# redradman/MujocoPoseLearning

Measured on AMD Instinct MI355X. Metric: env steps/sec (whole node), humanoid 'stand' task, 1/2/4/8 MI355X, higher is better.
Workload: dtype f64

## Files before the change

### mujocoposelearning_amd/csrc/hs_lanes.h

```cpp
#pragma once
#include <hip/hip_runtime.h>

#include <cstdint>
#include <type_traits>

#include "hs_kernels.h"
#include "hs_model.h"

namespace hs {
namespace {

constexpr int WAVE = 64;
constexpr int HL = 32;
static_assert(MAXDOF == HL, "one dof per sub-lane (lim_row slots, dof masks)");

template <int NCON, int NEFC, bool W = false, bool LT = false>
struct Cap {
  static constexpr int CON = NCON;
  static constexpr int EFC = NEFC;
  static constexpr int RPL = NEFC / HL;
  static constexpr bool WIDE = W;
  static constexpr bool LANES = LT;
  static constexpr bool NEAR = LT;
  static_assert((NCON % HL == 0 || HL % NCON == 0) && NEFC % HL == 0, "capacity in whole half-waves");
};
template <typename T>
using Resident = std::conditional_t<sizeof(T) == 8, Cap<MAXCON_F64, MAXEFC_F64, false, true>, Cap<MAXCON, MAXEFC>>;
using Wide = Cap<MAXCON_WIDE, MAXEFC_WIDE, true>;

#define SCHED_FENCE() __builtin_amdgcn_sched_barrier(0)

#define WSYNC() asm volatile("" ::: "memory")

template <int B, int E, typename F>
__device__ __forceinline__ void static_for(F&& f) {
  if constexpr (B < E) {
    f(std::integral_constant<int, B>{});
    static_for<B + 1, E>(f);
  }
}
template <int CTRL>
__device__ __forceinline__ uint32_t dpp32(uint32_t v) {
  return (uint32_t)__builtin_amdgcn_mov_dpp((int)v, CTRL, 0xF, 0xF, true);
}
struct RowPair { uint32_t lo, hi; };
__device__ __forceinline__ RowPair rowswap(uint32_t v) {
  auto r = __builtin_amdgcn_permlane16_swap(v, v, false, false);
  return {r[0], r[1]};
}
template <int K>
__device__ __forceinline__ uint32_t bcast32(uint32_t v) {
  RowPair r = rowswap(dpp32<0x150 + (K & 15)>(v));
  return K < 16 ? r.lo : r.hi;
}
template <int K>
__device__ __forceinline__ float bcast(float v) {
  return __uint_as_float(bcast32<K>(__float_as_uint(v)));
}
template <int K>
__device__ __forceinline__ double bcast(double v) {
  uint64_t x = (uint64_t)__double_as_longlong(v);
  uint64_t lo = bcast32<K>((uint32_t)x), hi = bcast32<K>((uint32_t)(x >> 32));
  return __longlong_as_double((long long)((hi << 32) | lo));
}
template <int CTRL>
__device__ __forceinline__ float dpp(float v) {
  return __uint_as_float(dpp32<CTRL>(__float_as_uint(v)));
}
template <int CTRL>
__device__ __forceinline__ double dpp(double v) {
  uint64_t x = (uint64_t)__double_as_longlong(v);
  uint64_t lo = dpp32<CTRL>((uint32_t)x), hi = dpp32<CTRL>((uint32_t)(x >> 32));
  return __longlong_as_double((long long)((hi << 32) | lo));
}
__device__ __forceinline__ float rows_sum(float v) {
  RowPair r = rowswap(__float_as_uint(v));
  return __uint_as_float(r.lo) + __uint_as_float(r.hi);
}
__device__ __forceinline__ double rows_sum(double v) {
  uint64_t x = (uint64_t)__double_as_longlong(v);
  RowPair l = rowswap((uint32_t)x), h = rowswap((uint32_t)(x >> 32));
  return __longlong_as_double((long long)(((uint64_t)h.lo << 32) | l.lo)) +
         __longlong_as_double((long long)(((uint64_t)h.hi << 32) | l.hi));
}
__device__ __forceinline__ float up_row(float v) { return __uint_as_float(rowswap(__float_as_uint(v)).hi); }
__device__ __forceinline__ double up_row(double v) {
  uint64_t x = (uint64_t)__double_as_longlong(v);
  const uint64_t lo = rowswap((uint32_t)x).hi, hi = rowswap((uint32_t)(x >> 32)).hi;
  return __longlong_as_double((long long)((hi << 32) | lo));
}
template <typename T>
__device__ __forceinline__ T hsum(T v) {
  v += dpp<0xB1>(v);
  v += dpp<0x4E>(v);
  v += dpp<0x141>(v);
  v += dpp<0x140>(v);
  return rows_sum(v);
}
__device__ __forceinline__ uint32_t hballot(bool p, bool upper) {
  uint64_t m = __ballot(p);
  return upper ? (uint32_t)(m >> 32) : (uint32_t)m;
}
template <typename T, bool AHEAD = false, typename LD, typename F>
__device__ __forceinline__ void for_bits(uint32_t mk, LD&& ld, F&& f) {
  if constexpr (AHEAD) {
    if (mk == 0u) return;
    int j = __builtin_ctz(mk);
    mk &= mk - 1u;
    auto cur = ld(j);
    for (; mk; mk &= mk - 1u) {
      const int jn = __builtin_ctz(mk);
      auto nxt = ld(jn);
      f(j, cur);
      cur = nxt;
      j = jn;
    }
    f(j, cur);
  } else {
    for (; mk; mk &= mk - 1u) {
      const int j = __builtin_ctz(mk);
      f(j, ld(j));
    }
  }
}
template <typename T, int N>
struct Vals { T v[N]; };
template <typename T, int N>
struct ValsX { T x; T v[N]; };

template <typename P>
__device__ __forceinline__ P opaque(P p) {
  uint64_t v = (uint64_t)p;
  uint32_t lo = __builtin_amdgcn_readfirstlane((uint32_t)v), hi = __builtin_amdgcn_readfirstlane((uint32_t)(v >> 32));
  v = ((uint64_t)hi << 32) | lo;
  asm volatile("" : "+s"(v));
  return (P)v;
}
template <typename T>
using MPtr = const __attribute__((address_space(4))) DevModel<T>*;
template <typename T>
using CPtr = const __attribute__((address_space(4))) T*;
template <typename T>
__device__ __forceinline__ LaneTable<T>& lane_table() {
  __shared__ LaneTable<T> tab;
  return tab;
}
template <typename T>
__device__ __forceinline__ void load_lane_table(MPtr<T> m) {
  constexpr int N = (int)(sizeof(LaneTable<T>) / 16), PER = (N + WAVE - 1) / WAVE;
  static_assert(sizeof(LaneTable<T>) % 16 == 0 && alignof(LaneTable<T>) == 16, "16-byte pieces");
  typedef uint32_t Piece __attribute__((ext_vector_type(4)));
  CPtr<Piece> src = (CPtr<Piece>)&m->lanes;
  Piece* dst = reinterpret_cast<Piece*>(&lane_table<T>());
  const int lane = threadIdx.x;
  Piece v[PER];
#pragma unroll
  for (int i = 0; i < PER; i++) {
    const int k = lane + i * WAVE;
    v[i] = src[k < N ? k : N - 1];
  }
#pragma unroll
  for (int i = 0; i < PER; i++) {
    const int k = lane + i * WAVE;
    if (k < N) dst[k] = v[i];
  }
  asm volatile("" ::: "memory");
}
template <typename C, typename T>
__device__ __forceinline__ decltype(auto) lanes(MPtr<T> m) {
  if constexpr (C::LANES) return (lane_table<T>());
  else return (*m);
}
#ifdef HS_ONLY_F32
#define HS_LT(C, m) (*(m))
#define HS_KTAIL(s) (s).u.k
#else
#define HS_LT(C, m) lanes<C>(m)
#define HS_KTAIL(s) (s).ktail()
#endif
template <typename T>
struct KArgs {
  MPtr<T> m;
  EnvBuffers<T> b;
  const float* actions;
  const uint8_t* reset_mask;
  const T* nz_q;
  const T* nz_v;
  StepParams p;
  int nenv;
  TapeOut<T> tape;
  RolloutArgs ro;
  EvalArgs ev;
  NormArgs nm;
  TermArgs tm;
};
template <typename T>
using KPtr = const __attribute__((address_space(4))) KArgs<T>*;
__device__ __forceinline__ int opaque_v(int x) {
  asm volatile("" : "+v"(x));
  return x;
}
__device__ __forceinline__ int below(uint32_t m, int sl) { return __popc(m & ((1u << sl) - 1u)); }
__device__ __forceinline__ bool bit(uint32_t mask, int i) { return i < 32 && ((mask >> i) & 1u); }
template <typename T>
__device__ __forceinline__ bool isbad(T x) {
  return !(x <= T(1e10) && x >= T(-1e10));
}

template <typename T>
__device__ __forceinline__ T row_ld(const T* p) {
  return __hip_atomic_load(const_cast<T*>(p), __ATOMIC_RELAXED, __HIP_MEMORY_SCOPE_AGENT);
}
template <typename T>
__device__ __forceinline__ void row_st(T* p, T v) {
  __hip_atomic_store(p, v, __ATOMIC_RELAXED, __HIP_MEMORY_SCOPE_AGENT);
}

__device__ __forceinline__ void sincos_t(double x, double& s, double& c) { sincos(x, &s, &c); }
__device__ __forceinline__ void sincos_t(float x, float& s, float& c) { s = __sinf(x); c = __cosf(x); }
template <typename T>
__device__ __forceinline__ void quat2mat(const T* q, T* R) {
  T w = q[0], x = q[1], y = q[2], z = q[3];
  R[0] = 1 - 2 * (y * y + z * z); R[1] = 2 * (x * y - w * z); R[2] = 2 * (x * z + w * y);
  R[3] = 2 * (x * y + w * z); R[4] = 1 - 2 * (x * x + z * z); R[5] = 2 * (y * z - w * x);
  R[6] = 2 * (x * z - w * y); R[7] = 2 * (y * z + w * x); R[8] = 1 - 2 * (x * x + y * y);
}
template <typename T>
__device__ __forceinline__ void mulq(const T* a, const T* b, T* r) {
  T t0 = a[0] * b[0] - a[1] * b[1] - a[2] * b[2] - a[3] * b[3];
  T t1 = a[0] * b[1] + a[1] * b[0] + a[2] * b[3] - a[3] * b[2];
  T t2 = a[0] * b[2] - a[1] * b[3] + a[2] * b[0] + a[3] * b[1];
  T t3 = a[0] * b[3] + a[1] * b[2] - a[2] * b[1] + a[3] * b[0];
  r[0] = t0; r[1] = t1; r[2] = t2; r[3] = t3;
}
template <typename T>
__device__ __forceinline__ void mv3(const T* R, const T* v, T* r) {
  T a = R[0] * v[0] + R[1] * v[1] + R[2] * v[2];
  T b = R[3] * v[0] + R[4] * v[1] + R[5] * v[2];
  T c = R[6] * v[0] + R[7] * v[1] + R[8] * v[2];
  r[0] = a; r[1] = b; r[2] = c;
}
template <typename T>
__device__ __forceinline__ void cross3(const T* a, const T* b, T* r) {
  T x = a[1] * b[2] - a[2] * b[1], y = a[2] * b[0] - a[0] * b[2], z = a[0] * b[1] - a[1] * b[0];
  r[0] = x; r[1] = y; r[2] = z;
}
template <typename T>
__device__ __forceinline__ T dot3(const T* a, const T* b) { return a[0] * b[0] + a[1] * b[1] + a[2] * b[2]; }
template <typename T>
__device__ __forceinline__ T dot6(const T* a, const T* b) {
  return a[0] * b[0] + a[1] * b[1] + a[2] * b[2] + a[3] * b[3] + a[4] * b[4] + a[5] * b[5];
}
template <typename T>
__device__ __forceinline__ T rsqrt_t(T x);
template <>
__device__ __forceinline__ float rsqrt_t<float>(float x) { return __builtin_amdgcn_rsqf(x); }
__device__ __forceinline__ float recip(float x) { return 1.0f / x; }
__device__ __forceinline__ double recip(double x) {
  double y = __builtin_amdgcn_rcp(x);
  const double e = fma(-x, y, 1.0);
  return fma(fma(e, e, e), y, y);
}
template <>
__device__ __forceinline__ double rsqrt_t<double>(double x) {
  const double y = __builtin_amdgcn_rsq(x);
  double g = x * y, h = 0.5 * y;
  const double r = fma(-h, g, 0.5);
  h = fma(h, r, h);
  const double y1 = h + h;
  const double e = fma(-(x * y1), y1, 1.0);
  return fma(h, e, y1);
}
template <typename T>
__device__ __forceinline__ T normalize3(T* v) {
  const T n2 = dot3(v, v);
  if (n2 < T(1e-30)) { v[0] = 1; v[1] = 0; v[2] = 0; return sqrt(n2); }
  const T i = rsqrt_t(n2);
  v[0] *= i; v[1] *= i; v[2] *= i;
  return n2 * i;
}
template <typename T>
__device__ __forceinline__ void normalize4(T* q) {
  const T n2 = q[0] * q[0] + q[1] * q[1] + q[2] * q[2] + q[3] * q[3];
  if (n2 < T(1e-30)) { q[0] = 1; q[1] = q[2] = q[3] = 0; }
  else { const T i = rsqrt_t(n2); q[0] *= i; q[1] *= i; q[2] *= i; q[3] *= i; }
}
template <typename T>
__device__ __forceinline__ void mul_inert(const T* i, const T* v, T* r) {
  r[0] = i[0] * v[0] + i[3] * v[1] + i[4] * v[2] - i[8] * v[4] + i[7] * v[5];
  r[1] = i[3] * v[0] + i[1] * v[1] + i[5] * v[2] + i[8] * v[3] - i[6] * v[5];
  r[2] = i[4] * v[0] + i[5] * v[1] + i[2] * v[2] - i[7] * v[3] + i[6] * v[4];
  r[3] = i[8] * v[1] - i[7] * v[2] + i[9] * v[3];
  r[4] = i[6] * v[2] - i[8] * v[0] + i[9] * v[4];
  r[5] = i[7] * v[0] - i[6] * v[1] + i[9] * v[5];
}
template <typename T>
__device__ __forceinline__ void cross_motion(const T* v, const T* m, T* r) {
  r[0] = -v[2] * m[1] + v[1] * m[2];
  r[1] = v[2] * m[0] - v[0] * m[2];
  r[2] = -v[1] * m[0] + v[0] * m[1];
  r[3] = -v[2] * m[4] + v[1] * m[5] - v[5] * m[1] + v[4] * m[2];
  r[4] = v[2] * m[3] - v[0] * m[5] + v[5] * m[0] - v[3] * m[2];
  r[5] = -v[1] * m[3] + v[0] * m[4] - v[4] * m[0] + v[3] * m[1];
}
template <typename T>
__device__ __forceinline__ void cross_force(const T* v, const T* f, T* r) {
  r[0] = -v[2] * f[1] + v[1] * f[2] - v[5] * f[4] + v[4] * f[5];
  r[1] = v[2] * f[0] - v[0] * f[2] + v[5] * f[3] - v[3] * f[5];
  r[2] = -v[1] * f[0] + v[0] * f[1] - v[4] * f[3] + v[3] * f[4];
  r[3] = -v[2] * f[4] + v[1] * f[5];
  r[4] = v[2] * f[3] - v[0] * f[5];
  r[5] = -v[1] * f[3] + v[0] * f[4];
}

}
}
```

### mujocoposelearning_amd/csrc/hs_scratch.h

```cpp
#pragma once
#include <cstdint>

#include "hs_lanes.h"
#include "hs_model.h"

namespace hs {
namespace {

enum RowKind { RK_JLO = 0, RK_JHI = 1, RK_TLO = 2, RK_THI = 3, RK_CN = 4, RK_P0 = 5 };
__device__ __forceinline__ int rk_kind(int kid) { return kid >> 16; }
__device__ __forceinline__ int rk_id(int kid) { return kid & 0xffff; }

template <typename T>
struct KinTail { T xanchor[MAXJNT][3]; T xaxis[MAXJNT][3]; T gpos[MAXGEOM][3]; T gax[MAXGEOM][3]; };

template <typename T, typename C>
struct Scratch {
  T qpos[MAXQ];
  T qvel[MAXDOF];
  T ctrl[MAXU];
  alignas(16) T vx[MAXDOF];
  T com[4];
  T cinert[MAXBODY][10];
  T cdof[MAXDOF][6];
  T cvel[MAXBODY][6];
  T con_pos[C::CON][3];
  T con_n[C::CON][3];
  T con_t1[C::CON][3];
  T con_dist[C::CON];
  T con_v[C::CON][3];
  T con_U[C::CON][6];
  T con_F[C::CON][3];
  int con_pair[C::CON];
  int con_adr[C::CON];
  uint32_t con_bb[C::CON];
  uint32_t con_m1[C::CON];
  uint32_t con_m2[C::CON];
  T con_mu[C::CON];
  uint32_t con_act[(C::CON + HL - 1) / HL];
  uint16_t lim_row[MAXDOF];
  uint32_t dense_mask[C::RPL];
  int row_kid[C::EFC];
  T row_D[C::EFC];
  T row_f[C::EFC];
  int ncon, nefc, nlim, njl;
  int niter;
  struct KinHead { T xpos[MAXBODY][3]; T xmat[MAXBODY][9]; T xquat[MAXBODY][4]; };
  struct KinFull { T xpos[MAXBODY][3]; T xmat[MAXBODY][9]; T xquat[MAXBODY][4]; T xanchor[MAXJNT][3];
                   T xaxis[MAXJNT][3]; T gpos[MAXGEOM][3]; T gax[MAXGEOM][3]; };
  using Kin = std::conditional_t<C::LANES, KinHead, KinFull>;
  static_assert(!C::LANES || sizeof(KinTail<T>) <= sizeof(T) * C::CON * 12, "KinTail fits con_v, con_U, con_F");
  __device__ __forceinline__ decltype(auto) ktail() {
    if constexpr (C::LANES) return (*reinterpret_cast<KinTail<T>*>(&con_v[0][0]));
    else return (u.k);
  }
  __device__ __forceinline__ decltype(auto) ktail() const {
    if constexpr (C::LANES) return (*reinterpret_cast<const KinTail<T>*>(&con_v[0][0]));
    else return (u.k);
  }
  static_assert(!C::NEAR || (C::LANES && sizeof(uint32_t) * MAXPAIR <= sizeof(T) * C::CON * 3 &&
                             sizeof(KinTail<T>) <= sizeof(T) * C::CON * 9),
                "the near-pair list fits con_F, past the KinTail over con_v / con_U");
  __device__ __forceinline__ uint32_t* near_list() { return reinterpret_cast<uint32_t*>(&con_F[0][0]); }
  union {
    Kin k;
    struct { T crb[MAXBODY][10]; T buf[MAXDOF][6]; } c;
    struct { T cdofdot[MAXDOF][6]; T cfrc[MAXBODY][6]; T csub[MAXBODY][6]; } r;
    struct { T bvel[MAXBODY][6];
             alignas(16) T cb[MAXDOF][2];
             T cfrc[MAXBODY][6], linv[MAXBODY][3], mv[MAXBODY][3]; } n;
    struct { alignas(16) float x[sizeof(T) == 8 ? 512 : 4]; alignas(16) float h[sizeof(T) == 8 ? 256 : 4]; } pol;
  } u;
};

constexpr int PGS_LA = 3;
template <typename T>
constexpr int pgs_cache_rows() { return sizeof(T) == 4 ? 40 : 48; }
template <typename T>
struct alignas(4 * sizeof(T)) PgsRow {
  T b, R, ar, ai;
  T g[4];
};
template <typename T, typename C>
struct PgsCache {
  static constexpr int NC = pgs_cache_rows<T>();
  T u[NC][MAXDOF];
  PgsRow<T> row[C::EFC];
};

}
}
```

### mujocoposelearning_amd/csrc/hs_stepper.h

```cpp
#pragma once
#include "hs_contacts.h"
#include "hs_dense.h"
#include "hs_lanes.h"
#include "hs_phase_clock.h"
#include "hs_scratch.h"

namespace hs {
namespace {

template <typename T, int NV, typename C>
struct Stepper {
  PhaseClock clk;
  MPtr<T> m;
  Scratch<T, C>& s;
  int sl, nb;
  bool up;
  T cd[6];
  T Mr[NV];
  T fsmooth;
  T fcon;
  T qacc;
  T qfa;
  T damp;
  int niter;
  T* dbg = nullptr;

  __device__ Stepper(MPtr<T> mm, Scratch<T, C>& ss, int lane)
      : m(mm), s(ss), sl(lane & (HL - 1)), nb(mm->nbody), up(lane >= HL) {}

  static constexpr bool LDLF = sizeof(T) == 8;
  static constexpr bool LDLE = false;
  __device__ __forceinline__ static KPtr<T> kargs() { return (KPtr<T>)__builtin_amdgcn_kernarg_segment_ptr(); }

  __device__ __forceinline__ void phase_begin() {
    m = opaque(m);
    sl = opaque_v(sl);
  }

  __device__ __forceinline__ void kinematics() {
    phase_begin();
    if (sl == 0) {
      for (int k = 0; k < 3; k++) s.u.k.xpos[0][k] = 0;
      s.u.k.xquat[0][0] = 1; s.u.k.xquat[0][1] = s.u.k.xquat[0][2] = s.u.k.xquat[0][3] = 0;
      for (int k = 0; k < 9; k++) s.u.k.xmat[0][k] = (k % 4 == 0) ? T(1) : T(0);
    }
    const int b = sl;
    const bool isb = b > 0 && b < nb;
    int depth = -1, par = 0, ja = 0, jn = 0, fqa = 0;
    bool isfree = false;
    T pl[3] = {0, 0, 0}, ql[4] = {1, 0, 0, 0};
    T anl[MAXJPB][3], axl[MAXJPB][3];
    if (isb) {
      depth = HS_LT(C, m).body_depth[b];
      par = HS_LT(C, m).body_parentid[b];
      ja = HS_LT(C, m).body_jntadr[b];
      jn = HS_LT(C, m).body_jntnum[b];
      isfree = jn == 1 && HS_LT(C, m).jnt_type[ja] == JNT_FREE;
      fqa = HS_LT(C, m).jnt_qposadr[ja];
      for (int k = 0; k < 3; k++) pl[k] = HS_LT(C, m).body_pos[b][k];
      for (int k = 0; k < 4; k++) ql[k] = HS_LT(C, m).body_quat[b][k];
    }
    if (isfree) {
      for (int k = 0; k < 3; k++) pl[k] = s.qpos[fqa + k];
      for (int k = 0; k < 4; k++) ql[k] = s.qpos[fqa + 3 + k];
    }
#pragma unroll
    for (int jj = 0; jj < MAXJPB; jj++) {
      const bool use = isb && !isfree && jj < jn;
      const int j = use ? ja + jj : 0;
      T jp[3], jx[3], ang = 0;
      for (int k = 0; k < 3; k++) { jp[k] = use ? m->jnt_pos[j][k] : T(0); jx[k] = use ? m->jnt_axis[j][k] : T(0); }
      if (use) {
        int qa = HS_LT(C, m).jnt_qposadr[j];
        ang = s.qpos[qa] - HS_LT(C, m).qpos0[qa];
      }
      T sn, cs;
      sincos_t(T(0.5) * ang, sn, cs);
      const T jr[4] = {cs, jx[0] * sn, jx[1] * sn, jx[2] * sn};
      T R[9];
      quat2mat(ql, R);
      mv3(R, jx, axl[jj]);
      mv3(R, jp, anl[jj]);
      for (int k = 0; k < 3; k++) anl[jj][k] += pl[k];
      if (use) {
        mulq(ql, jr, ql);
        quat2mat(ql, R);
        T v[3];
        mv3(R, jp, v);
        for (int k = 0; k < 3; k++) pl[k] = anl[jj][k] - v[k];
      }
    }
    WSYNC();
    for (int L = 1; L <= m->nlevel; L++) {
      if (depth == L) {
        T pos[3], q[4];
        if (isfree) {
          for (int k = 0; k < 3; k++) pos[k] = pl[k];
          for (int k = 0; k < 4; k++) q[k] = ql[k];
        } else {
          mv3(s.u.k.xmat[par], pl, pos);
          for (int k = 0; k < 3; k++) pos[k] += s.u.k.xpos[par][k];
          T pq[4] = {s.u.k.xquat[par][0], s.u.k.xquat[par][1], s.u.k.xquat[par][2], s.u.k.xquat[par][3]};
          mulq(pq, ql, q);
        }
        normalize4(q);
        for (int k = 0; k < 4; k++) s.u.k.xquat[b][k] = q[k];
        for (int k = 0; k < 3; k++) s.u.k.xpos[b][k] = pos[k];
        quat2mat(q, s.u.k.xmat[b]);
      }
      WSYNC();
    }
    if (isb) {
      if (isfree) {
        for (int k = 0; k < 3; k++) { HS_KTAIL(s).xanchor[ja][k] = s.u.k.xpos[b][k]; HS_KTAIL(s).xaxis[ja][k] = m->jnt_axis[ja][k]; }
      } else {
        const T* Rp = s.u.k.xmat[par];
        const T* xp = s.u.k.xpos[par];
#pragma unroll
        for (int jj = 0; jj < MAXJPB; jj++) {
          if (jj < jn) {
            T an[3], ax[3];
            mv3(Rp, anl[jj], an);
            mv3(Rp, axl[jj], ax);
            for (int k = 0; k < 3; k++) { HS_KTAIL(s).xanchor[ja + jj][k] = xp[k] + an[k]; HS_KTAIL(s).xaxis[ja + jj][k] = ax[k]; }
          }
        }
      }
    }
    if (sl < m->ngeom) {
      int g = sl, gb = HS_LT(C, m).geom_bodyid[g];
      T gp[3] = {m->geom_pos[g][0], m->geom_pos[g][1], m->geom_pos[g][2]};
      T gz[3] = {m->geom_zaxis[g][0], m->geom_zaxis[g][1], m->geom_zaxis[g][2]};
      T w[3];
      mv3(s.u.k.xmat[gb], gp, w);
      for (int k = 0; k < 3; k++) HS_KTAIL(s).gpos[g][k] = s.u.k.xpos[gb][k] + w[k];
      mv3(s.u.k.xmat[gb], gz, HS_KTAIL(s).gax[g]);
    }
    T mx = 0, my = 0, mz = 0, xi[3] = {0, 0, 0};
    if (b > 0 && b < nb) {
      T ip[3] = {m->body_ipos[b][0], m->body_ipos[b][1], m->body_ipos[b][2]}, w[3];
      mv3(s.u.k.xmat[b], ip, w);
      for (int k = 0; k < 3; k++) xi[k] = s.u.k.xpos[b][k] + w[k];
      T mb = HS_LT(C, m).body_mass[b];
      mx = mb * xi[0]; my = mb * xi[1]; mz = mb * xi[2];
    }
    T inv = T(1) / m->total_mass;
    T c0 = hsum(mx) * inv, c1 = hsum(my) * inv, c2 = hsum(mz) * inv;
    if (sl == 0) { s.com[0] = c0; s.com[1] = c1; s.com[2] = c2; }
    if (b > 0 && b < nb) {
      const T* R = s.u.k.xmat[b];
      CPtr<T> I6 = m->body_inert[b];
      T I[9] = {I6[0], I6[3], I6[4], I6[3], I6[1], I6[5], I6[4], I6[5], I6[2]};
      T A[9];
      for (int r = 0; r < 3; r++)
        for (int c = 0; c < 3; c++) A[3 * r + c] = R[3 * r] * I[c] + R[3 * r + 1] * I[3 + c] + R[3 * r + 2] * I[6 + c];
      T Ic[6];
      Ic[0] = A[0] * R[0] + A[1] * R[1] + A[2] * R[2];
      Ic[1] = A[3] * R[3] + A[4] * R[4] + A[5] * R[5];
      Ic[2] = A[6] * R[6] + A[7] * R[7] + A[8] * R[8];
      Ic[3] = A[0] * R[3] + A[1] * R[4] + A[2] * R[5];
      Ic[4] = A[0] * R[6] + A[1] * R[7] + A[2] * R[8];
      Ic[5] = A[3] * R[6] + A[4] * R[7] + A[5] * R[8];
      T d[3] = {xi[0] - c0, xi[1] - c1, xi[2] - c2};
      T mass = HS_LT(C, m).body_mass[b];
      T* ci = s.cinert[b];
      ci[0] = Ic[0] + mass * (d[1] * d[1] + d[2] * d[2]);
      ci[1] = Ic[1] + mass * (d[0] * d[0] + d[2] * d[2]);
      ci[2] = Ic[2] + mass * (d[0] * d[0] + d[1] * d[1]);
      ci[3] = Ic[3] - mass * d[0] * d[1];
      ci[4] = Ic[4] - mass * d[0] * d[2];
      ci[5] = Ic[5] - mass * d[1] * d[2];
      ci[6] = mass * d[0]; ci[7] = mass * d[1]; ci[8] = mass * d[2]; ci[9] = mass;
    }
    if (sl == 0)
      for (int k = 0; k < 10; k++) s.cinert[0][k] = 0;
    for (int k = 0; k < 6; k++) cd[k] = 0;
    if (sl < NV) {
      int j = HS_LT(C, m).dof_jntid[sl], db = HS_LT(C, m).dof_bodyid[sl];
      T off[3] = {c0 - HS_KTAIL(s).xanchor[j][0], c1 - HS_KTAIL(s).xanchor[j][1], c2 - HS_KTAIL(s).xanchor[j][2]};
      T ax[3];
      bool lin = false;
      if (HS_LT(C, m).jnt_type[j] == JNT_FREE) {
        int k = sl - HS_LT(C, m).jnt_dofadr[j];
        if (k < 3) {
          lin = true;
          cd[3] = k == 0 ? T(1) : T(0); cd[4] = k == 1 ? T(1) : T(0); cd[5] = k == 2 ? T(1) : T(0);
        } else {
          int c = k - 3;
          ax[0] = s.u.k.xmat[db][c]; ax[1] = s.u.k.xmat[db][3 + c]; ax[2] = s.u.k.xmat[db][6 + c];
        }
      } else {
        ax[0] = HS_KTAIL(s).xaxis[j][0]; ax[1] = HS_KTAIL(s).xaxis[j][1]; ax[2] = HS_KTAIL(s).xaxis[j][2];
      }
      if (!lin) {
        cd[0] = ax[0]; cd[1] = ax[1]; cd[2] = ax[2];
        cross3(ax, off, cd + 3);
      }
      for (int k = 0; k < 6; k++) s.cdof[sl][k] = cd[k];
    }
    WSYNC();
    if (dbg)
      for (int k = sl; k < MAXBODY * 3; k += HL) dbg[k] = s.u.k.xpos[k / 3][k % 3];
  }

  __device__ __forceinline__ int collision() {
    phase_begin();
    int ncon = 0;
    const int npair = m->npair;
    int4 info_n = make_int4(0, 0, 0, 0);
    T sz_n[4] = {0, 0, 0, 0};
    if (sl < npair) {
      info_n = make_int4(m->pair_info[sl][0], m->pair_info[sl][1], m->pair_info[sl][2], m->pair_info[sl][3]);
      for (int k = 0; k < 4; k++) sz_n[k] = m->pair_size[sl][k];
    }
    for (int base = 0; base < npair; base += HL) {
      int p = base + sl;
      Con<T> c0, c1;
      int n = 0;
      const int4 info = info_n;
      T sz[4] = {sz_n[0], sz_n[1], sz_n[2], sz_n[3]};
      if (p + HL < npair) {
        info_n = make_int4(m->pair_info[p + HL][0], m->pair_info[p + HL][1], m->pair_info[p + HL][2],
                           m->pair_info[p + HL][3]);
        for (int k = 0; k < 4; k++) sz_n[k] = m->pair_size[p + HL][k];
      }
      if (p < npair) n = collide_pair(s, info, sz, c0, c1);
      uint32_t m1 = hballot(n >= 1, up), m2 = hballot(n >= 2, up);
      int pre = below(m1, sl) + below(m2, sl);
      if (n >= 1) store_contact(m, s, ncon + pre, c0, p);
      if (n >= 2) store_contact(m, s, ncon + pre + 1, c1, p);
      ncon += __popc(m1) + __popc(m2);
    }
    int overflow = ncon > C::CON;
    if (overflow) ncon = C::CON;
    if (sl == 0) s.ncon = ncon;
    WSYNC();
    return overflow;
  }

  __device__ __forceinline__ int collision_near() {
    phase_begin();
    const int npair = m->npair;
    uint32_t* const list = s.near_list();
    int nlo = 0, nhi = 0;
    int4 info_n = make_int4(0, 0, 0, 0);
    T sz_n[4] = {0, 0, 0, 0};
    if (sl < npair) {
      info_n = make_int4(m->pair_info[sl][0], m->pair_info[sl][1], m->pair_info[sl][2], m->pair_info[sl][3]);
      for (int k = 0; k < 4; k++) sz_n[k] = m->pair_size[sl][k];
    }
    for (int base = 0; base < npair; base += HL) {
      const int p = base + sl;
      const int4 info = info_n;
      const T sz[4] = {sz_n[0], sz_n[1], sz_n[2], sz_n[3]};
      if (p + HL < npair) {
        info_n = make_int4(m->pair_info[p + HL][0], m->pair_info[p + HL][1], m->pair_info[p + HL][2],
                           m->pair_info[p + HL][3]);
        for (int k = 0; k < 4; k++) sz_n[k] = m->pair_size[p + HL][k];
      }
      const int g1 = info.x, g2 = info.y, fn = info.z;
      bool near = false;
      if (p < npair) {
        const T* p1 = HS_KTAIL(s).gpos[g1];
        const T* p2 = HS_KTAIL(s).gpos[g2];
        const T* a1 = HS_KTAIL(s).gax[g1];
        const T d[3] = {p2[0] - p1[0], p2[1] - p1[1], p2[2] - p1[2]};
        const T R = sz[0] + sz[1] + sz[2] + sz[3];
        const bool far_body = dot3(d, d) > R * R;
        const T reach = sz[2] + (fn == PAIR_PLANE_CAPSULE ? sz[3] : T(0));
        const bool far_plane = dot3(d, a1) > reach * T(1 + 1e-9) + T(1e-12);
        near = !(fn >= PAIR_SPHERE_SPHERE ? far_body : far_plane);
      }
      const uint64_t bm = __ballot(near);
      const uint32_t mk = up ? (uint32_t)(bm >> 32) : (uint32_t)bm;
      if (near) list[(up ? nhi : nlo) + below(mk, sl)] = near_entry(p, g1, g2, fn);
      nlo += __popc((uint32_t)bm);
      nhi += __popc((uint32_t)(bm >> 32));
    }
    const int nnear = up ? nhi : nlo;
    const int nmax = nlo > nhi ? nlo : nhi;
    WSYNC();
    int ncon = 0;
    for (int j0 = 0; j0 < nmax; j0 += HL) {
      const int j = j0 + sl;
      const bool on = j < nnear;
      const uint32_t e = on ? list[j] : 0u;
      const int p = e & 0xff, g1 = (e >> 8) & 0xff, g2 = (e >> 16) & 0xff, fn = e >> 24;
      const T sz[4] = {m->pair_size[p][0], m->pair_size[p][1], m->pair_size[p][2], m->pair_size[p][3]};
      const T mu = m->pair_mu[p];
      const int dim = m->pair_info[p][3];
      Con<T> c0, c1;
      int n = 0;
      if (on) n = collide_pair(s, make_int4(g1, g2, fn, dim), sz, c0, c1);
      uint32_t m1 = hballot(n >= 1, up), m2 = hballot(n >= 2, up);
      int pre = below(m1, sl) + below(m2, sl);
      if (n >= 1) store_contact_near(m, s, ncon + pre, c0, p, g1, g2, dim, mu);
      if (n >= 2) store_contact_near(m, s, ncon + pre + 1, c1, p, g1, g2, dim, mu);
      ncon += __popc(m1) + __popc(m2);
    }
    int overflow = ncon > C::CON;
    if (overflow) ncon = C::CON;
    if (sl == 0) s.ncon = ncon;
    WSYNC();
    return overflow;
  }

  __device__ __forceinline__ void mass_matrix() {
    phase_begin();
    if (sl > 0 && sl < nb) {
      const uint32_t dm = HS_LT(C, m).body_descmask[sl] & ~1u & ((nb < 32 ? (1u << nb) : 0u) - 1u);
      T a[10] = {0, 0, 0, 0, 0, 0, 0, 0, 0, 0};
      for_bits<T>(dm, [&](int c) { Vals<T, 10> r; for (int k = 0; k < 10; k++) r.v[k] = s.cinert[c][k]; return r; },
                  [&](int, const Vals<T, 10>& r) { for (int k = 0; k < 10; k++) a[k] += r.v[k]; });
      for (int k = 0; k < 10; k++) s.u.c.crb[sl][k] = a[k];
    }
    WSYNC();
    T bf[6] = {0, 0, 0, 0, 0, 0};
    uint32_t anci = 0;
    T arm = 0;
    if (sl < NV) {
      mul_inert(s.u.c.crb[HS_LT(C, m).dof_bodyid[sl]], cd, bf);
      for (int k = 0; k < 6; k++) s.u.c.buf[sl][k] = bf[k];
      anci = HS_LT(C, m).dof_ancmask[sl];
      arm = HS_LT(C, m).dof_armature[sl];
    }
    WSYNC();
    {
      T cb2[2][12];
      auto load = [&](auto jc, T (&dst)[12]) {
        constexpr int j = decltype(jc)::value;
        for (int k = 0; k < 6; k++) { dst[k] = s.cdof[j][k]; dst[6 + k] = s.u.c.buf[j][k]; }
      };
      load(std::integral_constant<int, 0>{}, cb2[0]);
      static_for<0, NV>([&](auto jc) {
        constexpr int j = decltype(jc)::value;
        if constexpr (j + 1 < NV) load(std::integral_constant<int, j + 1>{}, cb2[(j + 1) & 1]);
        SCHED_FENCE();
        const uint32_t ancj = m->dof_ancmask[j];
        const bool rel = (sl < NV) && (bit(anci, j) || bit(ancj, sl));
        const T* cj = cb2[j & 1];
        const T v = (j <= sl) ? dot6(cj, bf) : dot6(cd, cj + 6);
        Mr[j] = rel ? v + ((j == sl) ? arm : T(0)) : T(0);
      });
    }
    WSYNC();
  }

  __device__ __forceinline__ void velocity_forces() {
    phase_begin();
    if (sl < nb) {
      T v[6] = {0, 0, 0, 0, 0, 0};
      if (sl > 0) {
        const uint32_t ch = HS_LT(C, m).body_chainmask[sl];
        for_bits<T>(ch, [&](int j) { ValsX<T, 6> r; r.x = s.qvel[j]; for (int k = 0; k < 6; k++) r.v[k] = s.cdof[j][k]; return r; },
                    [&](int, const ValsX<T, 6>& r) { for (int k = 0; k < 6; k++) v[k] = fma(r.v[k], r.x, v[k]); });
      }
      for (int k = 0; k < 6; k++) s.cvel[sl][k] = v[k];
    }
    if (sl < NV) {
      const uint32_t dm = HS_LT(C, m).dof_dotmask[sl];
      T v[6] = {0, 0, 0, 0, 0, 0}, cdd[6];
      for_bits<T>(dm, [&](int j) { ValsX<T, 6> r; r.x = s.qvel[j]; for (int k = 0; k < 6; k++) r.v[k] = s.cdof[j][k]; return r; },
                  [&](int, const ValsX<T, 6>& r) { for (int k = 0; k < 6; k++) v[k] = fma(r.v[k], r.x, v[k]); });
      cross_motion(v, cd, cdd);
      for (int k = 0; k < 6; k++) s.u.r.cdofdot[sl][k] = cdd[k];
    }
    WSYNC();
    if (sl > 0 && sl < nb) {
      const uint32_t ch = HS_LT(C, m).body_chainmask[sl];
      T a[6] = {0, 0, 0, -m->gravity[0], -m->gravity[1], -m->gravity[2]};
      for_bits<T>(ch, [&](int j) { ValsX<T, 6> r; r.x = s.qvel[j]; for (int k = 0; k < 6; k++) r.v[k] = s.u.r.cdofdot[j][k]; return r; },
                  [&](int, const ValsX<T, 6>& r) { for (int k = 0; k < 6; k++) a[k] = fma(r.v[k], r.x, a[k]); });
      T f[6], t[6], t2[6];
      mul_inert(s.cinert[sl], a, f);
      mul_inert(s.cinert[sl], s.cvel[sl], t);
      cross_force(s.cvel[sl], t, t2);
      for (int k = 0; k < 6; k++) s.u.r.cfrc[sl][k] = f[k] + t2[k];
    }
    WSYNC();
    if (sl > 0 && sl < nb) {
      const uint32_t dm = HS_LT(C, m).body_descmask[sl] & ~1u & ((nb < 32 ? (1u << nb) : 0u) - 1u);
      T a[6] = {0, 0, 0, 0, 0, 0};
      for_bits<T>(dm, [&](int c) { Vals<T, 6> r; for (int k = 0; k < 6; k++) r.v[k] = s.u.r.cfrc[c][k]; return r; },
                  [&](int, const Vals<T, 6>& r) { for (int k = 0; k < 6; k++) a[k] += r.v[k]; });
      for (int k = 0; k < 6; k++) s.u.r.csub[sl][k] = a[k];
    }
    WSYNC();
    fsmooth = 0;
    qfa = 0;
    if (sl < NV) {
      T bias = dot6(cd, s.u.r.csub[HS_LT(C, m).dof_bodyid[sl]]);
      int qa = HS_LT(C, m).dof_qposadr[sl];
      T pas = -HS_LT(C, m).dof_damping[sl] * s.qvel[sl];
      if (qa >= 0) pas -= HS_LT(C, m).dof_stiffness[sl] * (s.qpos[qa] - HS_LT(C, m).dof_springref[sl]);
      int u = HS_LT(C, m).dof_actuator[sl];
      if (u >= 0) {
        T c = s.ctrl[u];
        if (HS_LT(C, m).act_ctrllimited[u]) c = fmin(HS_LT(C, m).act_ctrlrange[u][1], fmax(HS_LT(C, m).act_ctrlrange[u][0], c));
        qfa = HS_LT(C, m).act_gear[u] * c;
      }
      fsmooth = pas - bias + qfa;
    }
    WSYNC();
  }

  __device__ __forceinline__ int rows(T (&D)[C::RPL], T (&ar)[C::RPL], int (&rd)[C::RPL], T (&rc)[C::RPL]) {
    phase_begin();
    damp = sl < NV ? HS_LT(C, m).dof_damping[sl] : T(0);
    int overflow = 0;
    int ncon = s.ncon;
    int nrow = 0;
    {
      bool lo = false, hi = false;
      if (sl < m->njnt && HS_LT(C, m).jnt_limited[sl]) {
        T q = s.qpos[HS_LT(C, m).jnt_qposadr[sl]];
        lo = (q - HS_LT(C, m).jnt_range[sl][0]) < HS_LT(C, m).jnt_margin[sl];
        hi = (HS_LT(C, m).jnt_range[sl][1] - q) < HS_LT(C, m).jnt_margin[sl];
      }
      uint32_t ml = hballot(lo, up), mh = hballot(hi, up);
      int pre = below(ml, sl) + below(mh, sl);
      if (lo) s.row_kid[pre] = (RK_JLO << 16) | sl;
      if (hi) s.row_kid[pre + lo] = (RK_JHI << 16) | sl;
      nrow = __popc(ml) + __popc(mh);
      s.lim_row[sl] = 0;
      if (lo || hi)
        s.lim_row[HS_LT(C, m).jnt_dofadr[sl]] = (uint16_t)((lo ? pre + 1 : 0) | (hi ? (pre + lo + 1) << 8 : 0));
    }
    const int njl = nrow;
    {
      bool lo = false, hi = false;
      if (sl < m->ntendon && HS_LT(C, m).ten_limited[sl]) {
        T L = 0;
        for (int w = 0; w < HS_LT(C, m).ten_nwrap[sl]; w++) L += HS_LT(C, m).ten_wrapcoef[sl][w] * s.qpos[HS_LT(C, m).ten_wrapqadr[sl][w]];
        lo = (L - HS_LT(C, m).ten_range[sl][0]) < m->ten_margin[sl];
        hi = (HS_LT(C, m).ten_range[sl][1] - L) < m->ten_margin[sl];
      }
      uint32_t ml = hballot(lo, up), mh = hballot(hi, up);
      int pre = nrow + below(ml, sl) + below(mh, sl);
      if (lo) s.row_kid[pre] = (RK_TLO << 16) | sl;
      if (hi) s.row_kid[pre + lo] = (RK_THI << 16) | sl;
      nrow += __popc(ml) + __popc(mh);
    }
    int nlim = nrow;
    {
      int tot = 0;
#pragma unroll
      for (int cs = 0; cs < C::CON; cs += HL) {
        const int c = cs + sl;
        const bool isc = c < ncon;
        const bool pyr = isc && (s.con_bb[c] >> 16) == 3;
        tot += __popc(hballot(isc, up)) + 3 * __popc(hballot(pyr, up));
      }
      if (nrow + tot > C::EFC) {
        overflow = 1;
        int fit = 0, nr = nrow;
// ... 612 lines not shown
```

Before: 6.861 million.

## Precompute joint half-angle sincos per lane and hoist model loads in kinematics

In the lane-parallel kinematics path, each lane now computes sin/cos of the half joint angle for one joint and stores them in a new shared jsc array. The per-body joint loop reads these values instead of calling sincos serially for each joint. Model constants (joint pos/axis, geom pos/zaxis, body ipos/inertia) are loaded early into registers so their latency overlaps the computation, and the quaternion ops are rewritten with explicit FMAs. This adds a wave sync, extra scratch space and more register pressure, and the FMA forms change rounding slightly.

Result: no change. 6.918 million, median of 6 (+0.8%).

```diff
diff --git a/mujocoposelearning_amd/csrc/hs_lanes.h b/mujocoposelearning_amd/csrc/hs_lanes.h
--- a/mujocoposelearning_amd/csrc/hs_lanes.h
+++ b/mujocoposelearning_amd/csrc/hs_lanes.h
@@ -234,6 +234,32 @@
   r[0] = t0; r[1] = t1; r[2] = t2; r[3] = t3;
 }
 template <typename T>
+__device__ __forceinline__ void mulq_fma(const T* a, const T* b, T* r) {
+  const T t0 = fma(-a[3], b[3], fma(-a[2], b[2], fma(a[0], b[0], -(a[1] * b[1]))));
+  const T t1 = fma(-a[3], b[2], fma(a[2], b[3], fma(a[1], b[0], a[0] * b[1])));
+  const T t2 = fma(a[3], b[1], fma(a[2], b[0], fma(a[0], b[2], -(a[1] * b[3]))));
+  const T t3 = fma(a[3], b[0], fma(-a[2], b[1], fma(a[1], b[2], a[0] * b[3])));
+  r[0] = t0; r[1] = t1; r[2] = t2; r[3] = t3;
+}
+template <bool LATER, typename T>
+__device__ __forceinline__ void quat2mat_fma(const T* q, T* R) {
+  const T w = q[0], x = q[1], y = q[2], z = q[3];
+  const T wz = w * z, wy = w * y;
+  const T d0 = LATER ? fma(z, z, y * y) : fma(y, y, z * z);
+  const T d4 = LATER ? fma(z, z, x * x) : fma(x, x, z * z);
+  const T d8 = LATER ? fma(y, y, x * x) : fma(x, x, y * y);
+  R[0] = fma(d0, T(-2), T(1)); R[1] = 2 * fma(x, y, -wz); R[2] = 2 * fma(x, z, wy);
+  R[3] = 2 * fma(x, y, wz); R[4] = fma(d4, T(-2), T(1));
+  R[6] = 2 * fma(x, z, -wy); R[8] = fma(d8, T(-2), T(1));
+  if constexpr (LATER) {
+    const T wx = w * x;
+    R[5] = 2 * fma(y, z, -wx); R[7] = 2 * fma(y, z, wx);
+  } else {
+    const T yz = y * z;
+    R[5] = 2 * fma(-w, x, yz); R[7] = 2 * fma(w, x, yz);
+  }
+}
+template <typename T>
 __device__ __forceinline__ void mv3(const T* R, const T* v, T* r) {
   T a = R[0] * v[0] + R[1] * v[1] + R[2] * v[2];
   T b = R[3] * v[0] + R[4] * v[1] + R[5] * v[2];
diff --git a/mujocoposelearning_amd/csrc/hs_scratch.h b/mujocoposelearning_amd/csrc/hs_scratch.h
--- a/mujocoposelearning_amd/csrc/hs_scratch.h
+++ b/mujocoposelearning_amd/csrc/hs_scratch.h
@@ -45,7 +45,7 @@
   T row_f[C::EFC];
   int ncon, nefc, nlim, njl;
   int niter;
-  struct KinHead { T xpos[MAXBODY][3]; T xmat[MAXBODY][9]; T xquat[MAXBODY][4]; };
+  struct KinHead { T xpos[MAXBODY][3]; T xmat[MAXBODY][9]; T xquat[MAXBODY][4]; T jsc[MAXJNT][2]; };
   struct KinFull { T xpos[MAXBODY][3]; T xmat[MAXBODY][9]; T xquat[MAXBODY][4]; T xanchor[MAXJNT][3];
                    T xaxis[MAXJNT][3]; T gpos[MAXGEOM][3]; T gax[MAXGEOM][3]; };
   using Kin = std::conditional_t<C::LANES, KinHead, KinFull>;
diff --git a/mujocoposelearning_amd/csrc/hs_stepper.h b/mujocoposelearning_amd/csrc/hs_stepper.h
--- a/mujocoposelearning_amd/csrc/hs_stepper.h
+++ b/mujocoposelearning_amd/csrc/hs_stepper.h
@@ -64,6 +64,55 @@
       for (int k = 0; k < 3; k++) pl[k] = s.qpos[fqa + k];
       for (int k = 0; k < 4; k++) ql[k] = s.qpos[fqa + 3 + k];
     }
+#ifndef HS_ONLY_F32
+    [[maybe_unused]] T fax[3], gpl[3], gzl[3], ipl[3], I6l[6];
+    if constexpr (C::LANES) {
+      T jpl[MAXJPB][3], jxl[MAXJPB][3];
+      {
+        const int g = sl < m->ngeom ? sl : 0, bb = isb ? b : 0;
+        for (int jj = 0; jj < MAXJPB; jj++) {
+          const int j = (isb && !isfree && jj < jn) ? ja + jj : 0;
+          for (int k = 0; k < 3; k++) { jpl[jj][k] = m->jnt_pos[j][k]; jxl[jj][k] = m->jnt_axis[j][k]; }
+        }
+        for (int k = 0; k < 3; k++) {
+          fax[k] = m->jnt_axis[ja][k]; gpl[k] = m->geom_pos[g][k]; gzl[k] = m->geom_zaxis[g][k];
+          ipl[k] = m->body_ipos[bb][k];
+        }
+        for (int k = 0; k < 6; k++) I6l[k] = m->body_inert[bb][k];
+      }
+      if (sl < m->njnt) {
+        const int qa = HS_LT(C, m).jnt_qposadr[sl];
+        const T ang = HS_LT(C, m).jnt_type[sl] == JNT_FREE ? T(0) : s.qpos[qa] - HS_LT(C, m).qpos0[qa];
+        T sn, cs;
+        sincos_t(T(0.5) * ang, sn, cs);
+        s.u.k.jsc[sl][0] = sn; s.u.k.jsc[sl][1] = cs;
+      }
+      WSYNC();
+#pragma unroll
+      for (int jj = 0; jj < MAXJPB; jj++) {
+        const bool use = isb && !isfree && jj < jn;
+        const int j = use ? ja + jj : 0;
+        T jp[3], jx[3];
+        for (int k = 0; k < 3; k++) { jp[k] = use ? jpl[jj][k] : T(0); jx[k] = use ? jxl[jj][k] : T(0); }
+        const T sn = s.u.k.jsc[j][0], cs = s.u.k.jsc[j][1];
+        const T jr[4] = {cs, jx[0] * sn, jx[1] * sn, jx[2] * sn};
+        T R[9];
+        if (jj == 0) quat2mat_fma<false>(ql, R);
+        else quat2mat_fma<true>(ql, R);
+        mv3(R, jx, axl[jj]);
+        mv3(R, jp, anl[jj]);
+        for (int k = 0; k < 3; k++) anl[jj][k] += pl[k];
+        if (use) {
+          mulq_fma(ql, jr, ql);
+          quat2mat_fma<false>(ql, R);
+          T v[3];
+          mv3(R, jp, v);
+          for (int k = 0; k < 3; k++) pl[k] = anl[jj][k] - v[k];
+        }
+      }
+    } else
+#endif
+    {
 #pragma unroll
     for (int jj = 0; jj < MAXJPB; jj++) {
       const bool use = isb && !isfree && jj < jn;
@@ -90,6 +139,7 @@
         for (int k = 0; k < 3; k++) pl[k] = anl[jj][k] - v[k];
       }
     }
+    }
     WSYNC();
     for (int L = 1; L <= m->nlevel; L++) {
       if (depth == L) {
@@ -112,6 +162,11 @@
     }
     if (isb) {
       if (isfree) {
+#ifndef HS_ONLY_F32
+        if constexpr (C::LANES) {
+          for (int k = 0; k < 3; k++) { HS_KTAIL(s).xanchor[ja][k] = s.u.k.xpos[b][k]; HS_KTAIL(s).xaxis[ja][k] = fax[k]; }
+        } else
+#endif
         for (int k = 0; k < 3; k++) { HS_KTAIL(s).xanchor[ja][k] = s.u.k.xpos[b][k]; HS_KTAIL(s).xaxis[ja][k] = m->jnt_axis[ja][k]; }
       } else {
         const T* Rp = s.u.k.xmat[par];
@@ -131,6 +186,10 @@
       int g = sl, gb = HS_LT(C, m).geom_bodyid[g];
       T gp[3] = {m->geom_pos[g][0], m->geom_pos[g][1], m->geom_pos[g][2]};
       T gz[3] = {m->geom_zaxis[g][0], m->geom_zaxis[g][1], m->geom_zaxis[g][2]};
+#ifndef HS_ONLY_F32
+      if constexpr (C::LANES)
+        for (int k = 0; k < 3; k++) { gp[k] = gpl[k]; gz[k] = gzl[k]; }
+#endif
       T w[3];
       mv3(s.u.k.xmat[gb], gp, w);
       for (int k = 0; k < 3; k++) HS_KTAIL(s).gpos[g][k] = s.u.k.xpos[gb][k] + w[k];
@@ -139,6 +198,10 @@
     T mx = 0, my = 0, mz = 0, xi[3] = {0, 0, 0};
     if (b > 0 && b < nb) {
       T ip[3] = {m->body_ipos[b][0], m->body_ipos[b][1], m->body_ipos[b][2]}, w[3];
+#ifndef HS_ONLY_F32
+      if constexpr (C::LANES)
+        for (int k = 0; k < 3; k++) ip[k] = ipl[k];
+#endif
       mv3(s.u.k.xmat[b], ip, w);
       for (int k = 0; k < 3; k++) xi[k] = s.u.k.xpos[b][k] + w[k];
       T mb = HS_LT(C, m).body_mass[b];
@@ -151,6 +214,12 @@
       const T* R = s.u.k.xmat[b];
       CPtr<T> I6 = m->body_inert[b];
       T I[9] = {I6[0], I6[3], I6[4], I6[3], I6[1], I6[5], I6[4], I6[5], I6[2]};
+#ifndef HS_ONLY_F32
+      if constexpr (C::LANES) {
+        I[0] = I6l[0]; I[1] = I6l[3]; I[2] = I6l[4]; I[3] = I6l[3]; I[4] = I6l[1]; I[5] = I6l[5];
+        I[6] = I6l[4]; I[7] = I6l[5]; I[8] = I6l[2];
+      }
+#endif
       T A[9];
       for (int r = 0; r < 3; r++)
         for (int c = 0; c < 3; c++) A[3 * r + c] = R[3 * r] * I[c] + R[3 * r + 1] * I[3 + c] + R[3 * r + 2] * I[6 + c];
```
